# yynil/RWKVTTS

Hardware: AMD Instinct MI355X
Metric: audio-tokens/sec/GPU (train fwd+bwd) RWKV7-0.4B L=4096; 1->8 GPU scaling (higher is better)
Workload: dtype bf16; 1 GPU; RWKV7-0.4B Spark layout train step (fwd+bwd+AdamW), B=8/GPU L=4096, synthetic text+speech tokens, random init (BASELINE.json configs[1]); global_batch=8, seq_len=4096, parallelism=dp1, grad_allreduce=none

## Files before the change

include/rwkv7_hip.h:

```cpp
#ifndef RWKV7_HIP_H
#define RWKV7_HIP_H

#include <stddef.h>

#ifdef __cplusplus
extern "C" {
#endif

#define RWKV7_OK 0
#define RWKV7_EINVAL (-1)
#define RWKV7_ECHUNK (-2)
#define RWKV7_EHEAD  (-3)
#define RWKV7_ESHAPE (-4)

#define RWKV7_HEAD_SIZE 64
#define RWKV7_CHUNK_LEN 16

typedef void *rwkv7_stream_t;

const char *rwkv7_version(void);

int rwkv7_wkv_fwd_bf16(int B, int T, int H, const void *w, const void *q, const void *k, const void *v,
                       const void *a, const void *b, void *y, float *s, float *sa, rwkv7_stream_t stream);
int rwkv7_wkv_fwd_f32(int B, int T, int H, const void *w, const void *q, const void *k, const void *v,
// ... 133 lines not shown
                             const void *g, const void *gn_w, const void *gn_b, const void *r_k, float eps, void *out,
                             int nblocks, rwkv7_stream_t stream);
int rwkv7_tmix_post_fwd_f32(long rows, int D, const void *y, const void *r, const void *k, const void *v,
                            const void *g, const void *gn_w, const void *gn_b, const void *r_k, float eps, void *out,
                            int nblocks, rwkv7_stream_t stream);
int rwkv7_tmix_post_bwd_bf16(long rows, int D, const void *dout, const void *y, const void *r, const void *k,
                             const void *v, const void *g, const void *gn_w, const void *gn_b, const void *r_k,
                             float eps, void *d_y, void *d_r, void *d_k, void *d_v, void *d_g, float *dparams_partial,
                             int nblocks, rwkv7_stream_t stream);
int rwkv7_tmix_post_bwd_f32(long rows, int D, const void *dout, const void *y, const void *r, const void *k,
                            const void *v, const void *g, const void *gn_w, const void *gn_b, const void *r_k,
                            float eps, void *d_y, void *d_r, void *d_k, void *d_v, void *d_g, float *dparams_partial,
                            int nblocks, rwkv7_stream_t stream);
int rwkv7_tmix_post_bwd_compact_bf16(long rows, int D, const void *dout, const void *y, const void *r, const void *k,
                                     const void *v, const void *g, const void *gn_w, const void *gn_b, const void *r_k,
                                     float eps, void *d_y, void *dt, void *d_g, float *hscal, float *dparams_partial,
                                     int nblocks, rwkv7_stream_t stream);
int rwkv7_tmix_post_bwd_compact_f32(long rows, int D, const void *dout, const void *y, const void *r, const void *k,
                                    const void *v, const void *g, const void *gn_w, const void *gn_b, const void *r_k,
                                    float eps, void *d_y, void *dt, void *d_g, float *hscal, float *dparams_partial,
                                    int nblocks, rwkv7_stream_t stream);

int rwkv7_relusq_fwd_bf16(long n, const void *x, void *y, rwkv7_stream_t stream);
int rwkv7_relusq_fwd_f32(long n, const void *x, void *y, rwkv7_stream_t stream);
int rwkv7_relusq_bwd_bf16(long n, const void *x, const void *dy, void *dx, rwkv7_stream_t stream);
int rwkv7_relusq_bwd_f32(long n, const void *x, const void *dy, void *dx, rwkv7_stream_t stream);
int rwkv7_relusq_bwd_s_bf16(long n, const void *s, const void *dy, void *dx, rwkv7_stream_t stream);
int rwkv7_relusq_bwd_s_f32(long n, const void *s, const void *dy, void *dx, rwkv7_stream_t stream);

#define RWKV7_CHUNK_T 32
#define RWKV7_Q15_REC (64 * 64 + 2 * 256)
int rwkv7_wkv_chunk_prep_bf16(int B, int T, int H, const void *w, const void *a, const void *b, float *tinv,
                              rwkv7_stream_t stream);
int rwkv7_wkv_chunk_prep_f32(int B, int T, int H, const void *w, const void *a, const void *b, float *tinv,
                             rwkv7_stream_t stream);
int rwkv7_wkv_chunk_fwd_bf16(int B, int T, int H, const void *w, const void *q, const void *k, const void *v,
                             const void *a, const void *b, const float *tinv, void *y, float *sa, void *hs,
                             rwkv7_stream_t stream);
int rwkv7_wkv_chunk_fwd_f32(int B, int T, int H, const void *w, const void *q, const void *k, const void *v,
                            const void *a, const void *b, const float *tinv, void *y, float *sa, void *hs,
                            rwkv7_stream_t stream);
int rwkv7_wkv_chunk_fwd_seq_bf16(int B, int T, int H, const void *w, const void *q, const void *k, const void *v,
                                 const void *a, const void *b, const float *tinv, void *y, float *sa, void *hs,
                                 const int *seq_chunk_off, int nseq, rwkv7_stream_t stream);
int rwkv7_wkv_chunk_fwd_seq_f32(int B, int T, int H, const void *w, const void *q, const void *k, const void *v,
                                const void *a, const void *b, const float *tinv, void *y, float *sa, void *hs,
                                const int *seq_chunk_off, int nseq, rwkv7_stream_t stream);
int rwkv7_wkv_chunk_bseq_bf16(int B, int T, int H, const void *w, const void *q, const void *a, const void *b, const void *dy,
                              const float *tinv, void *e_vk, float *z, const int *seq_chunk_off, int nseq, rwkv7_stream_t stream);
int rwkv7_wkv_chunk_bwd_out_z_bf16(int B, int T, int H, const void *w, const void *q, const void *k, const void *v,
                                   const void *a, const void *b, const void *dy, const void *hs, const float *sa,
                                   const float *z, const void *e_vk, void *dw, void *dq, void *dk, void *dv,
                                   void *da, void *db, rwkv7_stream_t stream);
int rwkv7_wkv_chunk_fwd_state_bf16(int B, int T, int H, const void *w, const void *q, const void *k, const void *v,
                                   const void *a, const void *b, const float *tinv, void *y, float *sa, void *hs,
                                   const float *h0, float *hT, rwkv7_stream_t stream);
int rwkv7_wkv_chunk_bseq_state_bf16(int B, int T, int H, const void *w, const void *q, const void *a, const void *b,
                                    const void *dy, const float *tinv, void *e_vk, float *z,
                                    const float *dhT, float *dh0, rwkv7_stream_t stream);
int rwkv7_wkv_chunk_fwd_state_seq_bf16(int B, int T, int H, const void *w, const void *q, const void *k, const void *v,
                                       const void *a, const void *b, const float *tinv, void *y, float *sa, void *hs,
                                       const int *seq_chunk_off, int nseq, const float *h0, float *hT, rwkv7_stream_t stream);
int rwkv7_wkv_chunk_bseq_state_seq_bf16(int B, int T, int H, const void *w, const void *q, const void *a, const void *b,
                                        const void *dy, const float *tinv, void *e_vk, float *z, const int *seq_chunk_off, int nseq,
                                        const float *dhT, float *dh0, rwkv7_stream_t stream);
int rwkv7_ce_fwd_bwd_bf16(long rows, int V, void *logits, const long *labels, long ignore_index, float scale, float *loss_rows,
                          rwkv7_stream_t stream);
int rwkv7_ce_fwd_bwd_ls_bf16(long rows, int V, void *logits, const long *labels, long ignore_index, float scale, float *loss_rows,
                             float label_smoothing, rwkv7_stream_t stream);
int rwkv7_ce_fwd_bwd_ld_bf16(long rows, int V, long ld, void *logits, const long *labels, long ignore_index, float scale, float *loss_rows,
                             float label_smoothing, rwkv7_stream_t stream);

int rwkv7_adamw_bf16(long n, float *p32, const void *g16, float *m, float *v, void *p16, float lr, float beta1, float beta2,
                     float eps, float weight_decay, int step, rwkv7_stream_t stream);
int rwkv7_adamw_groups_bf16(long n, float *p32, const void *g16, float *m, float *v, void *p16, const unsigned char *slab_group,
                            const float *group_tab, int ngroups, const float *skip_flag, float lr, float beta1, float beta2,
                            float eps, int step, rwkv7_stream_t stream);

int rwkv7_sum_slabs_bf16(long n, int S, const float *parts, void *out, int accumulate, rwkv7_stream_t stream);
int rwkv7_transpose_bf16(int R, int C, const void *in, void *out, rwkv7_stream_t stream);
int rwkv7_gather_rows_bf16(long n_out, int D, const void *src, const int *idx, void *out, rwkv7_stream_t stream);
int rwkv7_wgrad_skinny_bf16(long M, int N, int K, int S, const void *dy, const void *x, float *parts, rwkv7_stream_t stream);
int rwkv7_wgrad_mid_bf16(long M, int N, int K, int S, const void *dy, const void *x, float *parts, rwkv7_stream_t stream);

int rwkv7_gemm_nt_bf16(int M, int N, int K, const void *A, const void *W, void *C, int epilogue, rwkv7_stream_t stream);
int rwkv7_gemm_nt_relusq_bwd_bf16(int M, int N, int K, const void *A, const void *W, const void *aux, void *C, rwkv7_stream_t stream);
int rwkv7_gemm_nt_relusq_bwd_s_bf16(int M, int N, int K, const void *A, const void *W, const void *s, void *C, rwkv7_stream_t stream);
int rwkv7_gemm_nt_add_bf16(int M, int N, int K, const void *A, const void *W, const void *resid, void *C, rwkv7_stream_t stream);

int rwkv7_mix_lora_wcat_fwd_bf16(int nb, const int *ranks, const void *const *w1, const void *const *mu, int D, void *wcat,
                                 rwkv7_stream_t stream);
int rwkv7_mix_lora_wcat_bwd_bf16(int nb, const int *ranks, const void *const *w1, const void *const *mu, int D, const void *dwcat,
                                 void *const *dw1, void *const *dmu, rwkv7_stream_t stream);
int rwkv7_mix_lora_combine_fwd_bf16(int nb, const int *ranks, const int *acts, long M, int T, const void *G, const void *mask,
                                    void *const *out, rwkv7_stream_t stream);
int rwkv7_mix_lora_combine_bwd_bf16(int nb, const int *ranks, const int *acts, long M, int T, const void *mask, const void *const *y,
                                    const void *const *dy, void *dG, rwkv7_stream_t stream);

int rwkv7_lora_down_pack_bf16(int nb, const int *ranks, const void *const *w1, int D, void *packed, rwkv7_stream_t stream);
int rwkv7_lora_down_fwd_bf16(int nb, const int *ranks, const int *acts, long M, int T, int D, const void *x, const void *mask,
                             const void *const *mu, const void *packed, void *const *out, rwkv7_stream_t stream);

int rwkv7_gemv32_bf16(int M, int N, int K, const void *x, const void *w, const void *bias, void *y, rwkv7_stream_t stream);

enum {
    RWKV7_DEC_LN0_W, RWKV7_DEC_LN0_B, RWKV7_DEC_LN1_W, RWKV7_DEC_LN1_B, RWKV7_DEC_LN2_W, RWKV7_DEC_LN2_B,
    RWKV7_DEC_XR, RWKV7_DEC_XW, RWKV7_DEC_XK, RWKV7_DEC_XV, RWKV7_DEC_XA, RWKV7_DEC_XG,
    RWKV7_DEC_WR, RWKV7_DEC_WK, RWKV7_DEC_WV, RWKV7_DEC_WO,
    RWKV7_DEC_W1, RWKV7_DEC_W2, RWKV7_DEC_W0, RWKV7_DEC_A1, RWKV7_DEC_A2, RWKV7_DEC_A0,
    RWKV7_DEC_V1, RWKV7_DEC_V2, RWKV7_DEC_V0, RWKV7_DEC_G1, RWKV7_DEC_G2,
    RWKV7_DEC_KK, RWKV7_DEC_KA, RWKV7_DEC_RK, RWKV7_DEC_GNW, RWKV7_DEC_GNB,
    RWKV7_DEC_FXK, RWKV7_DEC_WKEY, RWKV7_DEC_WVAL,
    RWKV7_DEC_ATT_XPREV, RWKV7_DEC_ATT_KV , RWKV7_DEC_FFN_XPREV,
    RWKV7_DEC_COUNT
};
typedef struct rwkv7_decode_dims {
    int B, D, H, L, F, V;
    int Rw, Ra, Rv, Rg;
    float ln_eps, gn_eps;
} rwkv7_decode_dims;
int rwkv7_decode_layer_ptrs(void);
size_t rwkv7_decode_workspace_bytes(const rwkv7_decode_dims *dims);
int rwkv7_decode_step_bf16(const rwkv7_decode_dims *dims, const void *const *layer_tbl, const void *x_in, const void *norm_w,
                           const void *norm_b, const void *head_w, const void *head_b, float *logits, void *workspace,
                           int persistent, rwkv7_stream_t stream);
int rwkv7_decode_step_tbl_bf16(const rwkv7_decode_dims *dims, const void *const *layer_tbl, const void *const *layer_tbl_host,
                               const void *x_in, const void *norm_w, const void *norm_b, const void *head_w, const void *head_b,
                               float *logits, void *workspace, int persistent, rwkv7_stream_t stream);

int rwkv7_sample_rows_f32(int rows, int nseg, const float *logits, long ld, const int *seg_off, const int *seg_len, const int *allow_lo,
                          const int *allow_hi, const int *suppress, int nsuppress, int max_domain, int do_sample, int top_k, float top_p,
                          float temperature, unsigned long long seed, const long *step, long *out, rwkv7_stream_t stream);
typedef struct rwkv7_sample_tail {
    unsigned char *unfinished;
    long eos, pad;
    long *ids;
    long *seq;
    long seq_ld;
    const void *emb;
    void *x;
    int D;
} rwkv7_sample_tail;
int rwkv7_sample_rows_tail_f32(int rows, const float *logits, long ld, const int *seg_off, const int *seg_len, const int *allow_lo,
                               const int *allow_hi, const int *suppress, int nsuppress, int max_domain, int do_sample, int top_k, float top_p,
                               float temperature, unsigned long long seed, const long *step, long *out, const rwkv7_sample_tail *tail,
                               int min_eos_id, long min_eos_until, rwkv7_stream_t stream);
typedef struct rwkv7_slot_state {
    long *step;
    long *limit;
    long *min_until;
    unsigned long long *seed;
    float *inv_temp;
    int *top_k;
    float *top_p;
    unsigned char *do_sample;
    unsigned char *live;
    long *ids;
    long *seq;
    long seq_ld;
    const void *emb;
    void *x;
    int D;
    int slots;
    int top_k_max;
    long eos;
} rwkv7_slot_state;
// ... 21 lines not shown
```

rwkvtts_amd/csrc/capi.hip:

```cpp
#include <hip/hip_runtime.h>
#include <math.h>

#include "../../include/rwkv7_hip.h"

namespace rwkv7 {
int wkv_fwd_bf16(int, int, int, const void *, const void *, const void *, const void *, const void *, const void *,
                 void *, float *, float *, float *, int, hipStream_t);
int wkv_fwd_f32(int, int, int, const void *, const void *, const void *, const void *, const void *, const void *,
                void *, float *, float *, float *, int, hipStream_t);
int wkv_bwd_bf16(int, int, int, const void *, const void *, const void *, const void *, const void *, const void *,
                 const void *, const float *, const float *, void *, void *, void *, void *, void *, void *,
                 hipStream_t);
int wkv_bwd_f32(int, int, int, const void *, const void *, const void *, const void *, const void *, const void *,
                const void *, const float *, const float *, void *, void *, void *, void *, void *, void *,
                hipStream_t);

int wkv_bwd_split_bf16(int, int, int, const void *, const void *, const void *, const void *, const void *, const void *,
                       const void *, const float *, const float *, void *const *, void *const *, void *const *, void *,
                       void *const *, void *const *, int, hipStream_t);
int wkv_bwd_split_f32(int, int, int, const void *, const void *, const void *, const void *, const void *, const void *,
                      const void *, const float *, const float *, void *const *, void *const *, void *const *, void *,
                      void *const *, void *const *, int, hipStream_t);
int chunk_prep_bf16(int, int, int, const void *, const void *, const void *, float *, hipStream_t);
int chunk_prep_f32(int, int, int, const void *, const void *, const void *, float *, hipStream_t);
int chunk_fwd_bf16(int, int, int, const void *, const void *, const void *, const void *, const void *, const void *,
                   const float *, void *, float *, void *, const int *, int, hipStream_t);
int chunk_fwd_f32(int, int, int, const void *, const void *, const void *, const void *, const void *, const void *,
                  const float *, void *, float *, void *, const int *, int, hipStream_t);
int chunk_debug_mma(const float *, const float *, float *, float *, hipStream_t);
int chunk_debug_tr16(const uint16_t *, const int *, uint16_t *, hipStream_t);
int gemv32_bf16(int, int, int, const void *, const void *, const void *, void *, hipStream_t);
int ce_fwd_bwd(long, int, long, void *, const long *, long, float, float *, float, hipStream_t);
int adamw_step(long, float *, const void *, float *, float *, void *, const uint8_t *, const float *, const float *, float, float, float, float,
               float, float, float, hipStream_t);
int lora32_bf16(int, int, int, int, int, const void *, const void *, const void *, const void *, void *, hipStream_t);
int chunk_bseq_bf16(int, int, int, const void *, const void *, const void *, const void *, const void *, const float *, void *,
                    float *, const int *, int, hipStream_t);
int chunk_bseq_state_seq_bf16(int, int, int, const void *, const void *, const void *, const void *, const void *, const float *,
                              void *, float *, const int *, int, const float *, float *, hipStream_t);
int chunk_fwd9_state_seq_bf16(int, int, int, const void *, const void *, const void *, const void *, const void *, const void *,
                              const float *, void *, float *, void *, const int *, int, const float *, float *, hipStream_t);
int gemm_nt4_bf16(int, int, int, const void *, const void *, void *, const void *, int, hipStream_t);
struct MixLoraDesc {
    int nb;
    int r[4], off[4];
    int act[4];
    const void *w1[4];
    const void *mu[4];
    void *out[4];
    void *out2[4];
};
int mix_lora_wcat_fwd(const MixLoraDesc &, int, int, void *, hipStream_t);
int mix_lora_wcat_bwd(const MixLoraDesc &, int, int, const void *, hipStream_t);
int mix_lora_combine_fwd(const MixLoraDesc &, long, int, int, const void *, const void *, hipStream_t);
int mix_lora_combine_bwd(const MixLoraDesc &, long, int, int, const void *, void *, hipStream_t);
struct LoraDownDesc {
    int nb;
    int r[4], off[4];
    int act[4];
    const void *w1[4];
    const void *mu[4];
    void *out[4];
    int tile0[5];
};
int lora_down_pack(const LoraDownDesc &, int, int, void *, hipStream_t);
int lora_down_fwd(LoraDownDesc &, int, long, int, int, const void *, const void *, const void *, hipStream_t);
int chunk_bwd_out10_bf16(int, int, int, const void *, const void *, const void *, const void *, const void *, const void *, const void *,
                         const void *, const float *, const float *, const void *, void *, void *, void *, void *, void *, void *, hipStream_t);
int sum_slabs_bf16(long, int, const float *, void *, int, hipStream_t);
int transpose_bf16(int, int, const void *, void *, hipStream_t);
int gather_rows16(long, int, const void *, const int *, void *, hipStream_t);
int wgrad_skinny_bf16(long, int, int, int, const void *, const void *, float *, hipStream_t);
int wgrad_mid_bf16(long, int, int, int, const void *, const void *, float *, hipStream_t);
int sample_rows_f32(int, int, const float *, long, const int *, const int *, const int *, const int *, const int *, int, int, int, int, float,
                    float, unsigned long long, const long *, long *, const void *, int, long, hipStream_t);
int sample_slots_f32(int, const float *, long, const int *, const int *, const int *, const int *, int, int, const void *, hipStream_t);
int ras_step_f32(int, const float *, long *, long *, long *, long *, long, int, float, int, int, float, unsigned long long, hipStream_t);
int xy_frame_step(int, int, int, long, long, long, long, long, const long *, int, int, const long *, long *, long *, long *, long *, long *,
                  unsigned char *, long *, hipStream_t);
int xy_embed_bf16(int, int, int, const void *const *, const long *, void *, hipStream_t);
int decode_layer_ptrs();
size_t decode_workspace_bytes(int, int, int, int, int, int, int, int, int);
int decode_step_bf16(int, int, int, int, int, int, int, int, int, int, float, float, const void *const *, const void *const *, const void *,
                     const void *, const void *, const void *, const void *, float *, void *, int, hipStream_t);
struct bf16_t;
template <typename T> int mix_fwd(int, int, int, int, const void *, const void *, const void *, const void *, void *, int, hipStream_t);
template <typename T> int mix_bwd(int, int, int, int, const void *const *, const void *, const void *, const void *, const void *, void *, float *, int, int, hipStream_t);
template <typename T> int tmix_prepare_fwd(long, int, const void *, const void *, const void *, const void *, const void *, const void *, const void *, const void *, const void *, void *, void *, void *, void *, void *, int, hipStream_t);
template <typename T> int tmix_prepare_bwd(long, int, const void *, const void *, const void *, const void *, const void *, const void *, const void *, const void *, const void *, const void *, const void *, const void *, const void *, const void *, void *, void *, void *, void *, void *, void *, float *, int, hipStream_t);
template <typename T> int tmix_prepare_bwd_sum(long, int, const void *, const void *, const void *, const void *, const void *, const void *, const void *, const void *, const void *, const void *const *, int, void *, void *, void *, void *, void *, void *, void *, float *, int, hipStream_t);
template <typename T> int tmix_post_fwd(long, int, const void *, const void *, const void *, const void *, const void *, const void *, const void *, const void *, float, void *, int, hipStream_t);
template <typename T> int tmix_post_bwd(long, int, const void *, const void *, const void *, const void *, const void *, const void *, const void *, const void *, const void *, float, void *, void *, void *, void *, void *, float *, float *, int, hipStream_t);
template <typename T> int add_ln_fwd(long, int, const void *, const void *, const void *, const void *, float, void *, void *, float *, float *, int, hipStream_t);
template <typename T> int add_ln_bwd(long, int, const void *, const void *, const void *, const float *, const float *, const void *, void *, float *, int, hipStream_t);
template <typename T> int add_ln_mix_fwd(int, int, int, int, void *, const void *, const void *, const void *, const void *, float, const void *, const void *, void *, void *, float *, float *, int, int, hipStream_t);
template <typename T> int mix_add_ln_bwd(int, int, int, int, const void *const *, const void *, const void *, const float *, const float *, const void *, const void *, const void *, const void *, void *, float *, int, int, hipStream_t);
template <typename T> int relusq_fwd(long, const void *, void *, hipStream_t);
template <typename T> int relusq_bwd(long, const void *, const void *, void *, hipStream_t);
template <typename T> int relusq_bwd_s(long, const void *, const void *, void *, hipStream_t);
}

namespace {
inline bool any_null(std::initializer_list<const void *> ps) {
    for (const void *p : ps)
        if (!p) return true;
    return false;
}
}

extern "C" {

const char *rwkv7_version(void) { return "rwkv7_hip 0.1.0 gfx950"; }

#define FWD_BODY(IMPL, CW)                                                                   \
    if (B <= 0 || T <= 0 || H <= 0 || any_null({w, q, k, v, a, b, y})) return RWKV7_EINVAL; \
    if ((s == nullptr) != (sa == nullptr)) return RWKV7_EINVAL;                              \
    if (T % RWKV7_CHUNK_LEN != 0) return RWKV7_ECHUNK;                                       \
    if ((CW) != 0 && (CW) != 4 && (CW) != 8) return RWKV7_ESHAPE;                            \
    return rwkv7::IMPL(B, T, H, w, q, k, v, a, b, y, s, sa, nullptr, CW, (hipStream_t)stream);

int rwkv7_wkv_fwd_bf16(int B, int T, int H, const void *w, const void *q, const void *k, const void *v,
                       const void *a, const void *b, void *y, float *s, float *sa, rwkv7_stream_t stream) {
    FWD_BODY(wkv_fwd_bf16, 0)
}
int rwkv7_wkv_fwd_f32(int B, int T, int H, const void *w, const void *q, const void *k, const void *v,
                      const void *a, const void *b, void *y, float *s, float *sa, rwkv7_stream_t stream) {
    FWD_BODY(wkv_fwd_f32, 0)
}
int rwkv7_wkv_fwd_variant_bf16(int B, int T, int H, const void *w, const void *q, const void *k, const void *v,
                               const void *a, const void *b, void *y, float *s, float *sa, int cols_per_lane, rwkv7_stream_t stream) {
    FWD_BODY(wkv_fwd_bf16, cols_per_lane)
}
int rwkv7_wkv_fwd_variant_f32(int B, int T, int H, const void *w, const void *q, const void *k, const void *v,
                              const void *a, const void *b, void *y, float *s, float *sa, int cols_per_lane, rwkv7_stream_t stream) {
    FWD_BODY(wkv_fwd_f32, cols_per_lane)
}

#define BWD_BODY(IMPL)                                                                                          \
    if (B <= 0 || T <= 0 || H <= 0 || any_null({w, q, k, v, a, b, dy, s, sa, dw, dq, dk, dv, da, db}))         \
        return RWKV7_EINVAL;                                                                                    \
    if (T % RWKV7_CHUNK_LEN != 0) return RWKV7_ECHUNK;                                                          \
    return rwkv7::IMPL(B, T, H, w, q, k, v, a, b, dy, s, sa, dw, dq, dk, dv, da, db, (hipStream_t)stream);

int rwkv7_wkv_bwd_bf16(int B, int T, int H, const void *w, const void *q, const void *k, const void *v,
                       const void *a, const void *b, const void *dy, const float *s, const float *sa, void *dw,
                       void *dq, void *dk, void *dv, void *da, void *db, rwkv7_stream_t stream) {
    BWD_BODY(wkv_bwd_bf16)
}
int rwkv7_wkv_bwd_f32(int B, int T, int H, const void *w, const void *q, const void *k, const void *v,
                      const void *a, const void *b, const void *dy, const float *s, const float *sa, void *dw,
                      void *dq, void *dk, void *dv, void *da, void *db, rwkv7_stream_t stream) {
    BWD_BODY(wkv_bwd_f32)
}

namespace {
constexpr size_t kArenaRec = (size_t)RWKV7_Q15_REC * 2, kArenaTinv = 32 * 32 * sizeof(float);
// ... 465 lines not shown
    if (D <= 0 || D % 128 != 0) return RWKV7_ESHAPE;
    for (int i = 0; i < nb; i++) {
        if (w1[i] == nullptr) return RWKV7_EINVAL;
        d.w1[i] = w1[i];
    }
    return rwkv7::lora_down_pack(d, R, D, packed, (hipStream_t)stream);
}
int rwkv7_lora_down_fwd_bf16(int nb, const int *ranks, const int *acts, long M, int T, int D, const void *x, const void *mask,
                             const void *const *mu, const void *packed, void *const *out, rwkv7_stream_t stream) {
    rwkv7::LoraDownDesc d;
    const int R = lora_down_desc(d, nb, ranks);
    if (R < 0) return R;
    if (acts == nullptr || x == nullptr || mu == nullptr || packed == nullptr || out == nullptr) return RWKV7_EINVAL;
    if (M <= 0 || T <= 0 || M % T != 0 || M % 128 != 0 || D <= 0 || D % 128 != 0 || D > 4096) return RWKV7_ESHAPE;
    for (int i = 0; i < nb; i++) {
        if (mu[i] == nullptr || out[i] == nullptr || acts[i] < 0 || acts[i] > 2) return RWKV7_EINVAL;
        d.act[i] = acts[i];
        d.mu[i] = mu[i];
        d.out[i] = out[i];
    }
    const int rc = rwkv7::lora_down_fwd(d, R, M, T, D, x, mask, packed, (hipStream_t)stream);
    return rc == -4 ? RWKV7_ESHAPE : rc;
}
int rwkv7_gemv32_bf16(int M, int N, int K, const void *x, const void *w, const void *bias, void *y, rwkv7_stream_t stream) {
    if (any_null({x, w, y})) return RWKV7_EINVAL;
    if (M <= 0 || M > 32 || N <= 0 || K <= 0 || K % 64 != 0) return RWKV7_ESHAPE;
    return rwkv7::gemv32_bf16(M, N, K, x, w, bias, y, (hipStream_t)stream);
}
int rwkv7_lora32_bf16(int M, int N, int K, int R, int act, const void *x, const void *w1, const void *w2, const void *bias,
                      void *y, rwkv7_stream_t stream) {
    if (any_null({x, w1, w2, y})) return RWKV7_EINVAL;
    if (M <= 0 || M > 32 || N <= 0 || K <= 0 || K % 64 != 0 || (R != 32 && R != 64 && R != 128) || act < 0 || act > 2)
        return RWKV7_ESHAPE;
    return rwkv7::lora32_bf16(M, N, K, R, act, x, w1, w2, bias, y, (hipStream_t)stream);
}
int rwkv7_adamw_groups_bf16(long n, float *p32, const void *g16, float *m, float *v, void *p16, const unsigned char *slab_group,
                            const float *group_tab, int ngroups, const float *skip_flag, float lr, float beta1, float beta2, float eps,
                            int step, rwkv7_stream_t stream) {
    if (n <= 0 || step <= 0 || any_null({(const void *)p32, g16, (const void *)m, (const void *)v, p16})) return RWKV7_EINVAL;
    if ((slab_group == nullptr) != (group_tab == nullptr) || (slab_group && (ngroups <= 0 || ngroups > 256))) return RWKV7_EINVAL;
    if (n % 4 != 0 || (slab_group && n % 128 != 0)) return RWKV7_ESHAPE;
    const double bc1 = 1.0 - pow((double)beta1, step), bc2 = 1.0 - pow((double)beta2, step);
    return rwkv7::adamw_step(n, p32, g16, m, v, p16, slab_group, group_tab, skip_flag, lr, beta1, beta2, eps, 0.f, (float)(1.0 / bc1),
                             (float)(1.0 / sqrt(bc2)), (hipStream_t)stream);
}
int rwkv7_adamw_bf16(long n, float *p32, const void *g16, float *m, float *v, void *p16, float lr, float beta1, float beta2,
                     float eps, float weight_decay, int step, rwkv7_stream_t stream) {
    if (n <= 0 || step <= 0 || any_null({(const void *)p32, g16, (const void *)m, (const void *)v, p16})) return RWKV7_EINVAL;
    if (n % 4 != 0) return RWKV7_ESHAPE;
    const double bc1 = 1.0 - pow((double)beta1, step), bc2 = 1.0 - pow((double)beta2, step);
    return rwkv7::adamw_step(n, p32, g16, m, v, p16, nullptr, nullptr, nullptr, lr, beta1, beta2, eps, weight_decay,
                             (float)(1.0 / bc1), (float)(1.0 / sqrt(bc2)), (hipStream_t)stream);
}
int rwkv7_ce_fwd_bwd_bf16(long rows, int V, void *logits, const long *labels, long ignore_index, float scale, float *loss_rows,
                          rwkv7_stream_t stream) {
    if (rows <= 0 || V <= 0 || any_null({(const void *)logits, (const void *)labels, (const void *)loss_rows})) return RWKV7_EINVAL;
    return rwkv7::ce_fwd_bwd(rows, V, V, logits, labels, ignore_index, scale, loss_rows, 0.f, (hipStream_t)stream);
}
int rwkv7_ce_fwd_bwd_ls_bf16(long rows, int V, void *logits, const long *labels, long ignore_index, float scale, float *loss_rows,
                             float label_smoothing,
                          rwkv7_stream_t stream) {
    if (rows <= 0 || V <= 0 || any_null({(const void *)logits, (const void *)labels, (const void *)loss_rows})) return RWKV7_EINVAL;
    if (!(label_smoothing >= 0.f && label_smoothing < 1.f)) return RWKV7_EINVAL;
    return rwkv7::ce_fwd_bwd(rows, V, V, logits, labels, ignore_index, scale, loss_rows, label_smoothing, (hipStream_t)stream);
}
int rwkv7_ce_fwd_bwd_ld_bf16(long rows, int V, long ld, void *logits, const long *labels, long ignore_index, float scale, float *loss_rows,
                             float label_smoothing, rwkv7_stream_t stream) {
    if (rows <= 0 || V <= 0 || ld < V || any_null({(const void *)logits, (const void *)labels, (const void *)loss_rows})) return RWKV7_EINVAL;
    if (!(label_smoothing >= 0.f && label_smoothing < 1.f)) return RWKV7_EINVAL;
    return rwkv7::ce_fwd_bwd(rows, V, ld, logits, labels, ignore_index, scale, loss_rows, label_smoothing, (hipStream_t)stream);
}
int rwkv7_wgrad_skinny_bf16(long M, int N, int K, int S, const void *dy, const void *x, float *parts, rwkv7_stream_t stream) {
    if (any_null({dy, x, parts})) return RWKV7_EINVAL;
    const int rank = N > K ? K : N, wide = N > K ? N : K;
    if (M <= 0 || S <= 0 || M % S != 0 || (M / S) % 128 != 0 || wide % 256 != 0 || (rank != 32 && rank != 64 && rank != 128))
        return RWKV7_ESHAPE;
    return rwkv7::wgrad_skinny_bf16(M, N, K, S, dy, x, parts, (hipStream_t)stream);
}
int rwkv7_wgrad_mid_bf16(long M, int N, int K, int S, const void *dy, const void *x, float *parts, rwkv7_stream_t stream) {
    if (any_null({dy, x, parts})) return RWKV7_EINVAL;
    if (M <= 0 || S <= 0 || M % S != 0 || (M / S) % 64 != 0 || K <= 0 || K % 256 != 0 || (N != 512 && N != 576)) return RWKV7_ESHAPE;
    return rwkv7::wgrad_mid_bf16(M, N, K, S, dy, x, parts, (hipStream_t)stream);
}
int rwkv7_sum_slabs_bf16(long n, int S, const float *parts, void *out, int accumulate, rwkv7_stream_t stream) {
    if (n <= 0 || S <= 0 || any_null({(const void *)parts, (const void *)out})) return RWKV7_EINVAL;
    if (n % 4 != 0) return RWKV7_ESHAPE;
    return rwkv7::sum_slabs_bf16(n, S, parts, out, accumulate, (hipStream_t)stream);
}
int rwkv7_gather_rows_bf16(long n_out, int D, const void *src, const int *idx, void *out, rwkv7_stream_t stream) {
    if (n_out <= 0 || D <= 0 || any_null({src, (const void *)idx, (const void *)out})) return RWKV7_EINVAL;
    if (D % 8 != 0) return RWKV7_ESHAPE;
    return rwkv7::gather_rows16(n_out, D, src, idx, out, (hipStream_t)stream);
}
int rwkv7_transpose_bf16(int R, int C, const void *in, void *out, rwkv7_stream_t stream) {
    if (R <= 0 || C <= 0 || any_null({in, (const void *)out})) return RWKV7_EINVAL;
    if (R % 64 != 0 || C % 64 != 0) return RWKV7_ESHAPE;
    return rwkv7::transpose_bf16(R, C, in, out, (hipStream_t)stream);
}
int rwkv7_decode_layer_ptrs(void) { return rwkv7::decode_layer_ptrs(); }
size_t rwkv7_decode_workspace_bytes(const rwkv7_decode_dims *dm) {
    if (!dm) return 0;
    return rwkv7::decode_workspace_bytes(dm->B, dm->D, dm->H, dm->F, dm->V, dm->Rw, dm->Ra, dm->Rv, dm->Rg);
}
int rwkv7_decode_step_bf16(const rwkv7_decode_dims *dm, const void *const *layer_tbl, const void *x_in, const void *norm_w,
                           const void *norm_b, const void *head_w, const void *head_b, float *logits, void *workspace,
                           int persistent, rwkv7_stream_t stream) {
    if (!dm || any_null({(const void *)layer_tbl, x_in, norm_w, norm_b, head_w, (const void *)logits, (const void *)workspace}))
        return RWKV7_EINVAL;
    if (dm->H * RWKV7_HEAD_SIZE != dm->D) return RWKV7_EHEAD;
    return rwkv7::decode_step_bf16(dm->B, dm->D, dm->H, dm->L, dm->F, dm->V, dm->Rw, dm->Ra, dm->Rv, dm->Rg, dm->ln_eps, dm->gn_eps,
                                   layer_tbl, nullptr, x_in, norm_w, norm_b, head_w, head_b, logits, workspace, persistent,
                                   (hipStream_t)stream);
}
int rwkv7_decode_step_tbl_bf16(const rwkv7_decode_dims *dm, const void *const *layer_tbl, const void *const *layer_tbl_host,
                               const void *x_in, const void *norm_w, const void *norm_b, const void *head_w, const void *head_b,
                               float *logits, void *workspace, int persistent, rwkv7_stream_t stream) {
    if (!dm || any_null({(const void *)layer_tbl, (const void *)layer_tbl_host, x_in, norm_w, norm_b, head_w, (const void *)logits,
                         (const void *)workspace}))
        return RWKV7_EINVAL;
    if (dm->H * RWKV7_HEAD_SIZE != dm->D) return RWKV7_EHEAD;
    return rwkv7::decode_step_bf16(dm->B, dm->D, dm->H, dm->L, dm->F, dm->V, dm->Rw, dm->Ra, dm->Rv, dm->Rg, dm->ln_eps, dm->gn_eps,
                                   layer_tbl, layer_tbl_host, x_in, norm_w, norm_b, head_w, head_b, logits, workspace, persistent,
                                   (hipStream_t)stream);
}
int rwkv7_sample_rows_f32(int rows, int nseg, const float *logits, long ld, const int *seg_off, const int *seg_len, const int *allow_lo,
                          const int *allow_hi, const int *suppress, int nsuppress, int max_domain, int do_sample, int top_k, float top_p,
                          float temperature, unsigned long long seed, const long *step, long *out, rwkv7_stream_t stream) {
    if (rows <= 0 || nseg <= 0 || max_domain <= 0 || nsuppress < 0 ||
        any_null({(const void *)logits, (const void *)seg_off, (const void *)seg_len, (const void *)step, (const void *)out}) ||
        (nsuppress > 0 && !suppress))
        return RWKV7_EINVAL;
    return rwkv7::sample_rows_f32(rows, nseg, logits, ld, seg_off, seg_len, allow_lo, allow_hi, suppress, nsuppress, max_domain, do_sample,
                                  top_k, top_p, temperature, seed, step, out, nullptr, -1, 0, (hipStream_t)stream);
}
int rwkv7_sample_rows_tail_f32(int rows, const float *logits, long ld, const int *seg_off, const int *seg_len, const int *allow_lo,
                               const int *allow_hi, const int *suppress, int nsuppress, int max_domain, int do_sample, int top_k, float top_p,
                               float temperature, unsigned long long seed, const long *step, long *out, const rwkv7_sample_tail *tail,
                               int min_eos_id, long min_eos_until, rwkv7_stream_t stream) {
    if (rows <= 0 || max_domain <= 0 || nsuppress < 0 ||
        any_null({(const void *)logits, (const void *)seg_off, (const void *)seg_len, (const void *)step, (const void *)out}) ||
        (nsuppress > 0 && !suppress))
        return RWKV7_EINVAL;
    return rwkv7::sample_rows_f32(rows, 1, logits, ld, seg_off, seg_len, allow_lo, allow_hi, suppress, nsuppress, max_domain, do_sample, top_k,
                                  top_p, temperature, seed, step, out, tail, min_eos_id, min_eos_until, (hipStream_t)stream);
}
int rwkv7_sample_slots_f32(int rows, const float *logits, long ld, const int *row_slot, const int *allow_lo, const int *allow_hi,
                           const int *suppress, int nsuppress, int max_domain, const rwkv7_slot_state *st, rwkv7_stream_t stream) {
    if (rows <= 0 || !st || !logits || max_domain <= 0 || nsuppress < 0 || (nsuppress > 0 && !suppress) || (!allow_lo != !allow_hi))
        return RWKV7_EINVAL;
    if (any_null({(const void *)st->step, (const void *)st->limit, (const void *)st->min_until, (const void *)st->seed,
                  (const void *)st->inv_temp, (const void *)st->top_k, (const void *)st->top_p, (const void *)st->do_sample,
                  (const void *)st->live, (const void *)st->ids, (const void *)st->seq}) ||
        st->seq_ld <= 0 || st->slots <= 0 || (st->emb && (!st->x || st->D <= 0)))
        return RWKV7_EINVAL;
    return rwkv7::sample_slots_f32(rows, logits, ld, row_slot, allow_lo, allow_hi, suppress, nsuppress, max_domain, st, (hipStream_t)stream);
}
int rwkv7_ras_step_f32(int V, const float *logits, long *tok, long *recent, long *ptr, long *step_i, long n_ignore, int eos, float top_p,
                       int top_k, int win_size, float tau_r, unsigned long long seed, rwkv7_stream_t stream) {
    if (V <= 0 || any_null({(const void *)logits, (const void *)tok, (const void *)recent, (const void *)ptr, (const void *)step_i}))
        return RWKV7_EINVAL;
    return rwkv7::ras_step_f32(V, logits, tok, recent, ptr, step_i, n_ignore, eos, top_p, top_k, win_size, tau_r, seed, (hipStream_t)stream);
}
int rwkv7_xy_frame_step(int B, int C, int rows, long text_shift, long speech_vocab, long pad, long eos0, long total, const long *eos_list,
                        int n_eos, int reference_termination, const long *nt, long *out, long *row, long *pos, long *unfinished, long *needs,
                        unsigned char *all_done, long *n_rows, rwkv7_stream_t stream) {
    if (B <= 0 || n_eos < 0 || (n_eos > 0 && !eos_list) ||
// ... 23 lines not shown
```

rwkvtts_amd/fused.py:

```python
import ctypes
import os

import torch

from . import _lib

_FWD_BLOCKS = 32768
_MIX_FWD_BLOCKS = 2048
_BWD_BLOCKS = 1024
_MIX_BWD_ROWS = 4
_MIX_BWD_BLOCKS = 1024


def _p(t):
    return None if t is None else ctypes.c_void_p(t.data_ptr())


def _stream(t):
    return ctypes.c_void_p(torch.cuda.current_stream(t.device).cuda_stream)


def _sfx(t):
    if not t.is_cuda:
        raise NotImplementedError("fused RWKV-7 stages run on the HIP device only (no CPU path)")
# ... 625 lines not shown
        else:
            d_y, d_r_post, d_k2_post, d_v2_post, d_g = [torch.empty_like(k) for _ in range(5)]
            _call("tmix_post_bwd", k, ctypes.c_long(rows), D, _p(dout), _p(y), _p(r), _p(k2), _p(v2), _p(g), _p(gn_w), _p(gn_b),
                  _p(r_k), ctypes.c_float(ctx.eps), _p(d_y), _p(d_r_post), _p(d_k2_post), _p(d_v2_post), _p(d_g),
                  _p(part_post), nb)
        if WGRAD_SYNC_BEFORE_SCAN:
            wgrad_side_sync(k.device)
        v4 = lambda t: t.view(B, T, H, 64)
        if ctx.chunked_fwd:
            dw, dq, dk, dv, da, db = ops.wkv7_chunk_backward(v4(w), v4(r), v4(k2), v4(v2), v4(a_in), v4(b_in), v4(d_y), s, sa,
                                                             tinv, seq_off=ctx.seq_start)
            dw2, dq2, dk2, da2, db2 = [(g, None) for g in (dw, dq, dk, da, db)]
        elif ctx.via_op:
            dw, dq, dk, dv, da, db = [torch.empty_like(k).view(B, T, H, 64) for _ in range(6)]
            torch.ops.wind_backstepping.backward(v4(w), v4(r), v4(k2), v4(v2), v4(a_in), v4(b_in), v4(d_y), s, sa, dw, dq, dk, dv, da, db)
            dw2, dq2, dk2, da2, db2 = [(g, None) for g in (dw, dq, dk, da, db)]
        else:
            dw2, dq2, dk2, dv, da2, db2 = ops.wkv7_backward_split(v4(w), v4(r), v4(k2), v4(v2), v4(a_in), v4(b_in),
                                                                  v4(d_y), s, sa)
        d_wpre, d_k, d_v, d_apre, d_r = [torch.empty_like(k) for _ in range(5)]
        d_vpre = torch.empty_like(k) if v_pre is not None else None
        d_vf = torch.empty_like(k) if v_pre is not None else None
        part = torch.empty(nb, 5, D, dtype=torch.float32, device=k.device)
        d_vf_next = None if (d_vf_next is None or v_pre is None) else _c(d_vf_next)
        gsum = [dw2[0], dw2[1], dk2[0], dk2[1], d_k2_post, dv, d_v2_post, da2[0], da2[1], db2[0], db2[1],
                dq2[0], dq2[1], d_r_post, d_vf_next]
        if compact:
            gsum += [dt_post, r, r_k, hscal]
        ptrs = (ctypes.c_void_p * len(gsum))(*[None if t is None else t.data_ptr() for t in gsum])
        _call("tmix_prepare_bwd_sum_compact" if compact else "tmix_prepare_bwd_sum", k, ctypes.c_long(rows), D, _p(w_pre), _p(k), _p(v), _p(a_pre), _p(v_pre), _p(v_first),
              _p(mask), _p(k_k), _p(k_a), ptrs, _p(d_wpre), _p(d_k), _p(d_v), _p(d_apre), _p(d_vpre), _p(d_vf),
              _p(d_r), _p(part), nb)
        dp = _colsum(part, k.dtype)
        dpp = _colsum(part_post, k.dtype)
        _attach_colsums(dp, d_wpre, d_apre, d_vpre)
        return (d_r, d_wpre, d_k, d_v, d_apre, d_g, d_vpre, d_vf, dp[0], dp[1], dpp[0], dpp[1], dpp[2], None, None,
                None, None)


def tmix_core(r, w_pre, k, v, a_pre, g, v_pre, v_first, k_k, k_a, gn_weight, gn_bias, r_k, mask, H, eps, is_layer0,
              seq_start=None):
    assert k.shape[-1] == H * 64
    if is_layer0:
        v_pre = v_first = None
    res = _TmixCore.apply(r, w_pre, k, v, a_pre, g, v_pre, v_first, k_k, k_a, gn_weight, gn_bias, r_k.reshape(-1),
                          _mask_rows(mask, k), H, eps, seq_start)
    if torch.is_tensor(res):
        return res, None
    return res


_ACT_ID = {None: 0, "tanh": 1, "sigmoid": 2}


def lora_decode_supported(x, rank):
    rows = x.numel() // x.shape[-1]
    return (GEMV_MAX_ROWS and x.is_cuda and x.dtype == torch.bfloat16 and rows <= GEMV_MAX_ROWS and rank in (32, 64, 128)
            and x.shape[-1] % 64 == 0 and not torch.is_grad_enabled())


def lora_decode(x, w1, w2, bias, activation):
    K, N, R = x.shape[-1], w2.shape[0], w1.shape[0]
    rows = x.numel() // K
    x2 = _c(x).view(rows, K)
    b2 = None if bias is None else _c(bias)
    y = torch.empty(rows, N, dtype=torch.bfloat16, device=x.device)
    with torch.cuda.device_of(x):
        rc = _lib.lib().rwkv7_lora32_bf16(rows, N, K, R, _ACT_ID[activation], _p(x2), _p(_c(w1)), _p(_c(w2)), _p(b2), _p(y),
                                          _stream(x))
    _lib.check(rc, "lora32")
    return y.view(*x.shape[:-1], N)


WGRAD_MIN_ROWS = 4096
WGRAD_SLABS_SMALL, WGRAD_SLABS_BIG = 8, 4
COMPACT_POST_BWD = True
SKINNY_WGRAD = True


MID_WGRAD = os.environ.get("RWKV7_MID_WGRAD", "1") == "1"
MID_WGRAD_SLABS = 32
MID_WGRAD_HITS = [0]


def wgrad_splitk(dy2, x2, out=None, slabs=None):
    M, N = dy2.shape
    K = x2.shape[1]
    rank, wide = min(N, K), max(N, K)
    if (SKINNY_WGRAD and dy2.dtype == torch.bfloat16 and x2.dtype == torch.bfloat16 and rank in (32, 64, 128) and wide % 256 == 0
            and M >= WGRAD_MIN_ROWS and M % 512 == 0):
        S = M // 512
        part = torch.empty(S, N, K, dtype=torch.float32, device=dy2.device)
        if out is None:
            out = torch.empty(N, K, dtype=torch.bfloat16, device=dy2.device)
        with torch.cuda.device_of(part):
            rc = _lib.lib().rwkv7_wgrad_skinny_bf16(ctypes.c_long(M), N, K, S, _p(dy2), _p(x2), _p(part), _stream(part))
            _lib.check(rc, "wgrad_skinny")
            rc = _lib.lib().rwkv7_sum_slabs_bf16(ctypes.c_long(N * K), S, _p(part), _p(out), 0, _stream(part))
        _lib.check(rc, "sum_slabs")
        return out
    if (MID_WGRAD and dy2.dtype == torch.bfloat16 and x2.dtype == torch.bfloat16 and N in (512, 576) and K % 256 == 0 and M >= WGRAD_MIN_ROWS
            and M % (MID_WGRAD_SLABS * 64) == 0 and dy2.is_contiguous() and x2.is_contiguous()):
        S = MID_WGRAD_SLABS
        part = torch.empty(S, N, K, dtype=torch.float32, device=dy2.device)
        if out is None:
            out = torch.empty(N, K, dtype=torch.bfloat16, device=dy2.device)
        with torch.cuda.device_of(part):
            rc = _lib.lib().rwkv7_wgrad_mid_bf16(ctypes.c_long(M), N, K, S, _p(dy2), _p(x2), _p(part), _stream(part))
            _lib.check(rc, "wgrad_mid")
            rc = _lib.lib().rwkv7_sum_slabs_bf16(ctypes.c_long(N * K), S, _p(part), _p(out), 0, _stream(part))
        _lib.check(rc, "sum_slabs")
        MID_WGRAD_HITS[0] += 1
        return out
    S = slabs if slabs else (WGRAD_SLABS_SMALL if N * K <= 1024 * 1024 else WGRAD_SLABS_BIG)
    if M < WGRAD_MIN_ROWS or M % (S * 8) != 0:
        res = torch.mm(dy2.t(), x2)
        if out is not None:
            out.copy_(res)
            return out
        return res
    part = torch.bmm(dy2.view(S, M // S, N).transpose(1, 2), x2.view(S, M // S, K), out_dtype=torch.float32)
    if dy2.dtype != torch.bfloat16 or (N * K) % 4 != 0:
        res = part.sum(0).to(dy2.dtype)
        if out is not None:
            out.copy_(res)
            return out
        return res
    if out is None:
        out = torch.empty(N, K, dtype=torch.bfloat16, device=dy2.device)
    with torch.cuda.device_of(part):
        rc = _lib.lib().rwkv7_sum_slabs_bf16(ctypes.c_long(N * K), S, _p(part), _p(out), 0, _stream(part))
    _lib.check(rc, "sum_slabs")
    return out


GATHER_ROWS_KERNEL = os.environ.get("RWKV7_GATHER_ROWS_KERNEL", "1") == "1"


class _GatherRows(torch.autograd.Function):

    @staticmethod
    def forward(ctx, src, idx, inv):
        src = _c(src)
        out = torch.empty(idx.numel(), src.shape[1], dtype=src.dtype, device=src.device)
        with torch.cuda.device_of(src):
            rc = _lib.lib().rwkv7_gather_rows_bf16(ctypes.c_long(idx.numel()), src.shape[1], _p(src), _p(idx), _p(out), _stream(src))
        _lib.check(rc, "gather_rows")
        ctx.save_for_backward(idx, inv)
        return out

    @staticmethod
    def backward(ctx, g):
        idx, inv = ctx.saved_tensors
        g = _c(g)
        dsrc = torch.empty(inv.numel(), g.shape[1], dtype=g.dtype, device=g.device)
        with torch.cuda.device_of(g):
            rc = _lib.lib().rwkv7_gather_rows_bf16(ctypes.c_long(inv.numel()), g.shape[1], _p(g), _p(inv), _p(dsrc), _stream(g))
        _lib.check(rc, "gather_rows(bwd)")
        return dsrc, None, None


def gather_rows(src, idx, inv):
    if (GATHER_ROWS_KERNEL and src.is_cuda and src.dtype == torch.bfloat16 and src.shape[1] % 8 == 0 and idx.dtype == torch.int32
            and inv.dtype == torch.int32):
        return _GatherRows.apply(src, idx, inv)
    out = src.index_select(0, idx.clamp(min=0).long())
    return out * (idx >= 0).unsqueeze(-1).to(out.dtype)


WGRAD_SIDE_STREAM = os.environ.get("RWKV7_WGRAD_SIDE_STREAM", "0") == "1"
WGRAD_SYNC_BEFORE_SCAN = False
_SIDE = {}


def wgrad_side_sync(device=None):
    for idx, ent in _SIDE.items():
        if ent[1] and (device is None or device.index == idx):
            torch.cuda.current_stream(ent[0].device).wait_stream(ent[0])
            ent[1] = False


def _wgrad(d2, x2, param):
    slot = _grad_slot(param)
    if slot is None:
        wgrad_side_sync(d2.device)
        return wgrad_splitk(d2, x2)
    if not WGRAD_SIDE_STREAM:
        wgrad_splitk(d2, x2, out=slot)
        return slot.view_as(param)
    ent = _SIDE.get(d2.device.index)
    if ent is None:
        ent = _SIDE[d2.device.index] = [torch.cuda.Stream(d2.device), False]
    side = ent[0]
    side.wait_stream(torch.cuda.current_stream(d2.device))
    with torch.cuda.stream(side):
        wgrad_splitk(d2, x2, out=slot)
# ... 392 lines not shown
```

Measured before the change: 273,800 tokens/s.

## Add custom split-K MFMA weight-gradient kernel for large square projections

Adds a dedicated HIP kernel that computes dy^T·x weight gradients for large N,K (multiples of 256). It uses double-buffered LDS staging, 32x32x16 bf16 MFMA, and an XCD-aware slab/tile assignment, then reduces fp32 slab partials with the existing sum_slabs kernel. This replaces the generic torch.bmm split-K path for those shapes. An optional ticket-based fused last-block reduction is included but disabled by default. The slab count is picked so tiles×slabs fills 256 workgroups, which is meant to improve occupancy and locality over the bmm path, at the cost of an fp32 partial buffer and a separate reduction pass.

```diff
diff --git a/include/rwkv7_hip.h b/include/rwkv7_hip.h
--- a/include/rwkv7_hip.h
+++ b/include/rwkv7_hip.h
@@ -239,6 +239,9 @@
 int rwkv7_gather_rows_bf16(long n_out, int D, const void *src, const int *idx, void *out, rwkv7_stream_t stream);
 int rwkv7_wgrad_skinny_bf16(long M, int N, int K, int S, const void *dy, const void *x, float *parts, rwkv7_stream_t stream);
 int rwkv7_wgrad_mid_bf16(long M, int N, int K, int S, const void *dy, const void *x, float *parts, rwkv7_stream_t stream);
+int rwkv7_wgrad_big_bf16(long M, int N, int K, int S, const void *dy, const void *x, float *parts, unsigned *tickets, void *out,
+                         rwkv7_stream_t stream);
+int rwkv7_wgrad_big_tiles(int N, int K, int S);
 
 int rwkv7_gemm_nt_bf16(int M, int N, int K, const void *A, const void *W, void *C, int epilogue, rwkv7_stream_t stream);
 int rwkv7_gemm_nt_relusq_bwd_bf16(int M, int N, int K, const void *A, const void *W, const void *aux, void *C, rwkv7_stream_t stream);
diff --git a/rwkvtts_amd/csrc/capi.hip b/rwkvtts_amd/csrc/capi.hip
--- a/rwkvtts_amd/csrc/capi.hip
+++ b/rwkvtts_amd/csrc/capi.hip
@@ -72,6 +72,8 @@
 int gather_rows16(long, int, const void *, const int *, void *, hipStream_t);
 int wgrad_skinny_bf16(long, int, int, int, const void *, const void *, float *, hipStream_t);
 int wgrad_mid_bf16(long, int, int, int, const void *, const void *, float *, hipStream_t);
+int wgrad_big_bf16(long, int, int, int, const void *, const void *, float *, unsigned *, void *, hipStream_t);
+int wgrad_big_tile_rows(int, int, int);
 int sample_rows_f32(int, int, const float *, long, const int *, const int *, const int *, const int *, const int *, int, int, int, int, float,
                     float, unsigned long long, const long *, long *, const void *, int, long, hipStream_t);
 int sample_slots_f32(int, const float *, long, const int *, const int *, const int *, const int *, int, int, const void *, hipStream_t);
@@ -703,6 +705,17 @@
     if (M <= 0 || S <= 0 || M % S != 0 || (M / S) % 64 != 0 || K <= 0 || K % 256 != 0 || (N != 512 && N != 576)) return RWKV7_ESHAPE;
     return rwkv7::wgrad_mid_bf16(M, N, K, S, dy, x, parts, (hipStream_t)stream);
 }
+int rwkv7_wgrad_big_bf16(long M, int N, int K, int S, const void *dy, const void *x, float *parts, unsigned *tickets, void *out,
+                         rwkv7_stream_t stream) {
+    if (any_null({dy, x, (const void *)parts}) || (tickets && !out)) return RWKV7_EINVAL;
+    if (M <= 0 || S <= 0 || M % S != 0 || (M / S) % 64 != 0 || N <= 0 || N % 256 != 0 || K <= 0 || K % 256 != 0) return RWKV7_ESHAPE;
+    if ((long)(N / 128) * (K / 256) * S > (1L << 20)) return RWKV7_ESHAPE;
+    return rwkv7::wgrad_big_bf16(M, N, K, S, dy, x, parts, tickets, out, (hipStream_t)stream);
+}
+int rwkv7_wgrad_big_tiles(int N, int K, int S) {
+    if (N <= 0 || K <= 0 || S <= 0 || N % 256 != 0 || K % 256 != 0) return RWKV7_ESHAPE;
+    return (N / rwkv7::wgrad_big_tile_rows(N, K, S)) * (K / 256);
+}
 int rwkv7_sum_slabs_bf16(long n, int S, const float *parts, void *out, int accumulate, rwkv7_stream_t stream) {
     if (n <= 0 || S <= 0 || any_null({(const void *)parts, (const void *)out})) return RWKV7_EINVAL;
     if (n % 4 != 0) return RWKV7_ESHAPE;
diff --git a/rwkvtts_amd/csrc/wgrad_big.hip b/rwkvtts_amd/csrc/wgrad_big.hip
--- /dev/null
+++ b/rwkvtts_amd/csrc/wgrad_big.hip
@@ -0,0 +1,189 @@
+#include "chunk_common.h"
+#include "launch_attr.h"
+
+namespace rwkv7 {
+
+namespace {
+constexpr int kBigLdX = 288;
+__host__ __device__ constexpr int big_ld_y(int nta) { return 64 * nta + 32; }
+__host__ __device__ constexpr int big_buf(int nta) { return 32 * (big_ld_y(nta) + kBigLdX); }
+
+constexpr int kBigStep = 32;
+
+template <int NTA>
+__global__ __launch_bounds__(512) void wgrad_big_kernel(int N, int K, int S, int rows_per_slab, const bf16_t *__restrict__ dy_,
+                                                        const bf16_t *__restrict__ x_, float *part, unsigned *tickets, uint16_t *out) {
+    constexpr int TM = 64 * NTA, LDY = big_ld_y(NTA), BUF = big_buf(NTA);
+    extern __shared__ __attribute__((aligned(16))) uint16_t sm[];
+    const int tid = threadIdx.x, lane = tid & 63;
+    const int wave = __builtin_amdgcn_readfirstlane(tid >> 6), cg = wave & 3, rh = wave >> 2;
+    const int ncb = K / 256, tiles = (N / TM) * ncb;
+    int slab, tile;
+    {
+        const int xcd = blockIdx.x & 7, j = blockIdx.x >> 3;
+        if ((S & 7) == 0) {
+            slab = (j / tiles) * 8 + xcd;
+            tile = j % tiles;
+        } else if (8 % S == 0 && tiles % (8 / S) == 0) {
+            const int g = 8 / S, per = tiles / g;
+            slab = xcd / g;
+            tile = (xcd % g) * per + j;
+        } else {
+            slab = blockIdx.x / tiles;
+            tile = blockIdx.x % tiles;
+        }
+    }
+    const int tn = tile / ncb, tk = tile % ncb;
+    const long row0 = (long)slab * rows_per_slab;
+    const uint16_t *xg = reinterpret_cast<const uint16_t *>(x_) + row0 * K + tk * 256;
+    const uint16_t *yg = reinterpret_cast<const uint16_t *>(dy_) + row0 * N + tn * TM;
+    const int xrow = tid >> 5, xcol = (tid & 31) * 8;
+    const int yrow = NTA == 4 ? tid >> 5 : tid >> 4, ycol = NTA == 4 ? (tid & 31) * 8 : (tid & 15) * 8;
+    const int nsteps = rows_per_slab / kBigStep;
+    struct Regs { uint4 x0, x1, y0, y1; };
+    auto fetch = [&](int step) {
+        Regs r;
+        step = step < nsteps ? step : nsteps - 1;
+        const uint16_t *xp = xg + ((long)step * kBigStep + xrow) * K + xcol, *yp = yg + ((long)step * kBigStep + yrow) * N + ycol;
+        r.x0 = *reinterpret_cast<const uint4 *>(xp);
+        r.x1 = *reinterpret_cast<const uint4 *>(xp + 16L * K);
+        r.y0 = *reinterpret_cast<const uint4 *>(yp);
+        if (NTA == 4) r.y1 = *reinterpret_cast<const uint4 *>(yp + 16L * N);
+        return r;
+    };
+    auto stage = [&](const Regs r, int b) {
+        uint16_t *sy = sm + b * BUF + yrow * LDY + ycol, *sx = sm + b * BUF + kBigStep * LDY + xrow * kBigLdX + xcol;
+        *reinterpret_cast<uint4 *>(sx) = r.x0;
+        *reinterpret_cast<uint4 *>(sx + 16 * kBigLdX) = r.x1;
+        *reinterpret_cast<uint4 *>(sy) = r.y0;
+        if (NTA == 4) *reinterpret_cast<uint4 *>(sy + 16 * LDY) = r.y1;
+    };
+    f32x16 acc[NTA][2];
+#pragma unroll
+    for (int i = 0; i < NTA; i++) acc[i][0] = acc[i][1] = zero16();
+    auto products = [&](int b) {
+        const uint16_t *sy = sm + b * BUF, *sx = sy + kBigStep * LDY;
+#pragma unroll
+        for (int ks = 0; ks < kBigStep / 16; ks++) {
+            bf16x8 yf[NTA], xf[2];
+#pragma unroll
+            for (int j = 0; j < 2; j++) xf[j] = frag_tr(sx, kBigLdX, 16 * ks, cg * 64 + j * 32, lane);
+#pragma unroll
+            for (int i = 0; i < NTA; i++) yf[i] = frag_tr(sy, LDY, 16 * ks, rh * (TM / 2) + i * 32, lane);
+            __builtin_amdgcn_sched_barrier(0);
+#pragma unroll
+            for (int i = 0; i < NTA; i++)
+#pragma unroll
+                for (int j = 0; j < 2; j++) acc[i][j] = __builtin_amdgcn_mfma_f32_32x32x16_bf16(yf[i], xf[j], acc[i][j], 0, 0, 0);
+        }
+    };
+#define WGB_STEP(R_, B_, AHEAD_)                                                                                       \
+    stage(R_, 1 - (B_));     \
+    __builtin_amdgcn_sched_barrier(0);                                                                               \
+    R_ = fetch(step + (AHEAD_));                                                                                     \
+    __builtin_amdgcn_sched_barrier(0);                                                                               \
+    products(B_);                                                                                                    \
+    lds_barrier();
+    Regs r0 = fetch(0), r1 = fetch(1);
+    stage(r0, 0);
+    r0 = fetch(2);
+    lds_barrier();
+    for (int step = 0; step < nsteps; step += 2) {
+        WGB_STEP(r1, 0, 3)
+        WGB_STEP(r0, 1, 4)
+    }
+#undef WGB_STEP
+    const int nbase0 = tn * TM + rh * (TM / 2), kbase0 = tk * 256 + cg * 64;
+    if (tickets == nullptr) {
+        float *p = part + (long)slab * N * K;
+#pragma unroll
+        for (int i = 0; i < NTA; i++)
+#pragma unroll
+            for (int j = 0; j < 2; j++)
+#pragma unroll
+                for (int r = 0; r < 16; r++) p[(long)(nbase0 + i * 32 + d_row(r, lane)) * K + kbase0 + j * 32 + (lane & 31)] = acc[i][j][r];
+        return;
+    }
+    constexpr int NV = NTA * 2 * 4;
+    float4 *pt = reinterpret_cast<float4 *>(part) + (long)tile * S * NV * 512 + tid;
+    {
+        float4 *p = pt + (long)slab * NV * 512;
+#pragma unroll
+        for (int i = 0; i < NTA; i++)
+#pragma unroll
+            for (int j = 0; j < 2; j++)
+#pragma unroll
+                for (int q = 0; q < 4; q++)
+                    p[((i * 2 + j) * 4 + q) * 512] = make_float4(acc[i][j][4 * q], acc[i][j][4 * q + 1], acc[i][j][4 * q + 2], acc[i][j][4 * q + 3]);
+    }
+    asm volatile("s_waitcnt vmcnt(0)" ::: "memory");
+    __syncthreads();
+    unsigned *flag = reinterpret_cast<unsigned *>(sm);
+    if (tid == 0) {
+        __builtin_amdgcn_fence(__ATOMIC_RELEASE, "agent");
+        asm volatile("s_waitcnt vmcnt(0)" ::: "memory");
+        const unsigned t = __hip_atomic_fetch_add(tickets + tile, 1u, __ATOMIC_RELAXED, __HIP_MEMORY_SCOPE_AGENT);
+        const unsigned last = t == (unsigned)(S - 1);
+        if (last) {
+            __builtin_amdgcn_fence(__ATOMIC_ACQUIRE, "agent");
+            asm volatile("s_waitcnt vmcnt(0)" ::: "memory");
+        }
+        *flag = last;
+    }
+    __syncthreads();
+    if (*flag == 0) return;
+    for (int i = 0; i < NTA; i++) {
+        float4 sum[8];
+#pragma unroll
+        for (int v = 0; v < 8; v++) sum[v] = make_float4(0.f, 0.f, 0.f, 0.f);
+        const float4 *p = pt + (long)i * 8 * 512;
+#pragma unroll 2
+        for (int s = 0; s < S; s++, p += (long)NV * 512) {
+            float4 t[8];
+#pragma unroll
+            for (int v = 0; v < 8; v++) t[v] = p[v * 512];
+#pragma unroll
+            for (int v = 0; v < 8; v++) {
+                sum[v].x += t[v].x;
+                sum[v].y += t[v].y;
+                sum[v].z += t[v].z;
+                sum[v].w += t[v].w;
+            }
+        }
+#pragma unroll
+        for (int j = 0; j < 2; j++)
+#pragma unroll
+            for (int q = 0; q < 4; q++) {
+                const float4 v = sum[j * 4 + q];
+                uint16_t *o = out + (long)(nbase0 + i * 32 + d_row(4 * q, lane)) * K + kbase0 + j * 32 + (lane & 31);
+                o[0] = f2bf(v.x);
+                o[(long)K] = f2bf(v.y);
+                o[2L * K] = f2bf(v.z);
+                o[3L * K] = f2bf(v.w);
+            }
+    }
+    if (tid == 0) __hip_atomic_store(tickets + tile, 0u, __ATOMIC_RELAXED, __HIP_MEMORY_SCOPE_AGENT);
+}
+
+template <int NTA>
+int launch_big(int grid, int N, int K, int S, int rows_per_slab, const void *dy, const void *x, float *part, unsigned *tickets, void *out,
+               hipStream_t st) {
+    constexpr int lds = big_buf(NTA) * 2 * 2;
+    static DynLdsOnce lds_once;
+    auto kern = &wgrad_big_kernel<NTA>;
+    if (hipError_t e = lds_once.ensure(reinterpret_cast<const void *>(kern), lds); e != hipSuccess) return (int)e;
+    (void)hipGetLastError();
+    kern<<<dim3((unsigned)grid), dim3(512), lds, st>>>(N, K, S, rows_per_slab, (const bf16_t *)dy, (const bf16_t *)x, part, tickets, (uint16_t *)out);
+    return (int)hipGetLastError();
+}
+}
+
+int wgrad_big_tile_rows(int N, int K, int S) { return (long)(N / 128) * (K / 256) * S <= 256 ? 128 : 256; }
+
+int wgrad_big_bf16(long M, int N, int K, int S, const void *dy, const void *x, float *parts, unsigned *tickets, void *out, hipStream_t st) {
+    const int rows_per_slab = (int)(M / S);
+    if (wgrad_big_tile_rows(N, K, S) == 128) return launch_big<2>((N / 128) * (K / 256) * S, N, K, S, rows_per_slab, dy, x, parts, tickets, out, st);
+    return launch_big<4>((N / 256) * (K / 256) * S, N, K, S, rows_per_slab, dy, x, parts, tickets, out, st);
+}
+
+}
diff --git a/rwkvtts_amd/fused.py b/rwkvtts_amd/fused.py
--- a/rwkvtts_amd/fused.py
+++ b/rwkvtts_amd/fused.py
@@ -731,6 +731,35 @@
 MID_WGRAD_SLABS = 32
 MID_WGRAD_HITS = [0]
 
+BIG_WGRAD = os.environ.get("RWKV7_BIG_WGRAD", "1") == "1"
+BIG_WGRAD_FUSED_REDUCE = False
+BIG_WGRAD_WGS = 256
+BIG_WGRAD_HITS = [0]
+_BIG_WS = {}
+
+
+def _big_wgrad_slabs(M, N, K):
+    if N % 256 or K % 256:
+        return 0
+    tiles = (N // 256) * (K // 256)
+    S = BIG_WGRAD_WGS // tiles if tiles <= BIG_WGRAD_WGS else 0
+    if S == 0 or S > 16 or tiles * S != BIG_WGRAD_WGS:
+        return 0
+    if S == 16:
+        S = 8
+    return S if M % (S * 64) == 0 else 0
+
+
+def _big_workspace(dev, stream, n_part, n_tickets):
+    ws = _BIG_WS.get((dev.index, stream))
+    if ws is None:
+        ws = _BIG_WS[(dev.index, stream)] = [torch.zeros(1024, dtype=torch.int32, device=dev), None]
+    if ws[0].numel() < n_tickets:
+        ws[0] = torch.zeros(n_tickets, dtype=torch.int32, device=dev)
+    if ws[1] is None or ws[1].numel() < n_part:
+        ws[1] = torch.empty(n_part, dtype=torch.float32, device=dev)
+    return ws
+
 
 def wgrad_splitk(dy2, x2, out=None, slabs=None):
     M, N = dy2.shape
@@ -761,6 +790,25 @@
         _lib.check(rc, "sum_slabs")
         MID_WGRAD_HITS[0] += 1
         return out
+    if (BIG_WGRAD and dy2.dtype == torch.bfloat16 and x2.dtype == torch.bfloat16 and M >= WGRAD_MIN_ROWS and dy2.is_cuda
+            and dy2.is_contiguous() and x2.is_contiguous() and (out is None or out.is_contiguous()) and _big_wgrad_slabs(M, N, K)):
+        S = _big_wgrad_slabs(M, N, K)
+        if out is None:
+            out = torch.empty(N, K, dtype=torch.bfloat16, device=dy2.device)
+        with torch.cuda.device_of(dy2):
+            st = _stream(dy2)
+            if BIG_WGRAD_FUSED_REDUCE:
+                tickets, part = _big_workspace(dy2.device, int(st.value or 0), S * N * K, _lib.lib().rwkv7_wgrad_big_tiles(N, K, S))
+                rc = _lib.lib().rwkv7_wgrad_big_bf16(ctypes.c_long(M), N, K, S, _p(dy2), _p(x2), _p(part), _p(tickets), _p(out), st)
+                _lib.check(rc, "wgrad_big")
+            else:
+                part = torch.empty(S, N, K, dtype=torch.float32, device=dy2.device)
+                rc = _lib.lib().rwkv7_wgrad_big_bf16(ctypes.c_long(M), N, K, S, _p(dy2), _p(x2), _p(part), None, None, st)
+                _lib.check(rc, "wgrad_big")
+                rc = _lib.lib().rwkv7_sum_slabs_bf16(ctypes.c_long(N * K), S, _p(part), _p(out), 0, st)
+                _lib.check(rc, "sum_slabs")
+        BIG_WGRAD_HITS[0] += 1
+        return out
     S = slabs if slabs else (WGRAD_SLABS_SMALL if N * K <= 1024 * 1024 else WGRAD_SLABS_BIG)
     if M < WGRAD_MIN_ROWS or M % (S * 8) != 0:
         res = torch.mm(dy2.t(), x2)
```

After: 276,800 tokens/s, median of 6. 1.01x the previous value.
